# kadircet/ceng795

Measured on AMD Instinct MI355X. Metric: Mrays/s at 1920×1080 (primary+shadow); fraction of HBM roofline, higher is better.
Workload: dtype f32; 1 GPU; C3: 999,698-triangle height field, 1920x1080, 1 point light, primary + shadow rays (BASELINE.json configs[2]); frame=1920x1080, triangles=999698, traversal=fast, parallelism=frames1, frames_in_flight=6

## Files before the change

ceng795_amd/_lib.py:

```python
from __future__ import annotations

import ctypes as C
import os

_HERE = os.path.dirname(os.path.abspath(__file__))
_VARIANT = os.environ.get("CENG795_LIB", "")
LIB_PATH = os.path.join(_HERE, "lib", f"libceng795_rt_{_VARIANT}.so" if _VARIANT else
                        "libceng795_rt.so")

RT_OK = 0
RT_E_INVALID = -1
RT_E_HIP = -2
RT_E_IO = -3
RT_E_PARSE = -4
RT_E_UNSUPPORTED = -5

RT_TRAVERSAL_FAST = 0
RT_TRAVERSAL_REFERENCE = 1

RT_QUERY_REORDER = 1
RT_QUERY_IN_MEDIUM = 2
RT_QUERY_LIGHTS_SHARED = 4
RT_QUERY_NO_SCENE_LIGHTS = 8
RT_QUERY_RAY_TIME = 32
# ... 115 lines not shown
    "rt_set_msaa_seed": (C.c_int, [C.c_void_p, C.c_ulonglong]),
    "rt_render": (C.c_int, [C.c_void_p, C.c_int, C.c_int, C.c_int, C.c_void_p,
                            C.POINTER(rt_stats)]),
    "rt_render_device": (C.c_int, [C.c_void_p, C.c_int, C.c_int, C.c_int, C.c_int, C.c_int,
                                   C.c_int, C.c_void_p, C.c_void_p]),
    "rt_render_device_range": (C.c_int, [C.c_void_p, C.c_int, C.c_int, C.c_int, C.c_int,
                                         C.c_int, C.c_int, C.c_int, C.c_void_p, C.c_void_p]),
    "rt_scene_records_ok": (C.c_int, [C.c_void_p, C.c_int]),
    "rt_tile_costs": (C.c_int, [C.c_void_p, C.c_void_p, C.c_void_p, C.c_int]),
    "rt_resolve_rows": (C.c_int, [C.c_void_p, C.c_int, C.c_int, C.c_int, C.c_void_p, C.c_void_p,
                                  C.c_void_p]),
    "rt_resolve_device": (C.c_int, [C.c_void_p, C.c_int, C.c_int, C.c_int, C.c_int, C.c_int,
                                    C.c_int, C.c_int, C.c_void_p, C.c_void_p, C.c_void_p]),
    "rt_set_kernel_timing": (C.c_int, [C.c_void_p, C.c_int]),
    "rt_read_kernel_times": (C.c_int, [C.c_void_p, C.POINTER(C.c_double),
                                       C.POINTER(C.c_longlong)]),
    "rt_num_tiles": (C.c_int, [C.c_void_p, C.c_int, C.c_int, C.c_int]),
    "rt_collect_stats": (C.c_int, [C.c_void_p, C.POINTER(rt_stats)]),
    "rt_write_png": (C.c_int, [C.c_char_p, C.c_void_p, C.c_int, C.c_int]),
    "rt_camera_from_view": (C.c_int, [C.POINTER(C.c_float), C.POINTER(C.c_float),
                                      C.POINTER(C.c_float), C.POINTER(C.c_float), C.c_float,
                                      C.c_int, C.c_int, C.c_int, C.POINTER(rt_camera)]),
    "rt_last_error": (C.c_char_p, []),
    "rt_abi_version": (C.c_int, []),
    "rt_host_dump_bvh_xml": (C.c_int, [C.c_char_p, C.c_char_p]),
    "rt_host_dump_bvh_desc": (C.c_int, [C.POINTER(rt_scene_desc), C.c_char_p]),
    "rt_host_alloc": (C.c_void_p, [C.c_size_t]),
    "rt_host_free": (None, [C.c_void_p]),
    "rt_host_check_accel_xml": (C.c_int, [C.c_char_p, C.c_int, C.POINTER(C.c_longlong)]),
    "rt_host_accel_slots_check": (C.c_int, [C.c_longlong, C.c_longlong]),
    "rt_host_packet_div": (C.c_int, [C.c_int, C.c_int, C.c_int, C.c_void_p]),
    "rt_host_packet_coords": (C.c_int, [C.c_int] * 8 + [C.c_void_p]),
    "rt_host_accel_slot_hist_xml": (C.c_int, [C.c_char_p, C.c_int, C.POINTER(C.c_longlong)]),
    "rt_debug_counters": (C.c_int, [C.c_void_p, C.POINTER(C.c_longlong)]),
    "rt_debug_timeline": (C.c_longlong, [C.POINTER(C.c_ulonglong), C.c_longlong]),
    "rt_debug_phases": (C.c_longlong, [C.POINTER(C.c_ulonglong), C.c_longlong]),
    "rt_debug_frame_occupancy": (C.c_int, [C.c_int, C.POINTER(C.c_int)]),
    "rt_debug_quotient_check": (C.c_int, [C.c_int, C.c_ulonglong, C.c_longlong,
                                          C.POINTER(C.c_longlong)]),
    "rt_debug_quotient_check_mode": (C.c_int, [C.c_int, C.c_int, C.c_ulonglong, C.c_longlong,
                                               C.POINTER(C.c_longlong)]),
    "rt_ray_query_version": (C.c_int, []),
    "rt_trace_rays_device": (C.c_int, [C.c_void_p, C.c_void_p, C.c_longlong, C.c_void_p, C.c_int,
                                       C.c_void_p]),
    "rt_occluded_device": (C.c_int, [C.c_void_p, C.c_void_p, C.c_longlong, C.c_void_p, C.c_int,
                                     C.c_void_p]),
    "rt_trace_rays": (C.c_int, [C.c_void_p, C.c_void_p, C.c_longlong, C.c_void_p, C.c_int]),
    "rt_occluded": (C.c_int, [C.c_void_p, C.c_void_p, C.c_longlong, C.c_void_p, C.c_int]),
    "rt_host_leaf_objects_desc": (C.c_int, [C.POINTER(rt_scene_desc), C.POINTER(C.c_int), C.c_int]),
    "rt_radiance_query_version": (C.c_int, []),
    "rt_shade_rays_device": (C.c_int, [C.c_void_p, C.c_void_p, C.c_longlong, C.c_int, C.c_void_p,
                                       C.c_int, C.c_void_p]),
    "rt_shade_rays": (C.c_int, [C.c_void_p, C.c_void_p, C.c_longlong, C.c_int, C.c_void_p, C.c_int,
                                C.POINTER(rt_stats)]),
    "rt_set_radiance_scratch_limit": (C.c_int, [C.c_void_p, C.c_size_t]),
    "rt_stream_frame_scratch_bytes": (C.c_longlong, [C.c_void_p, C.c_void_p]),
    "rt_film_version": (C.c_int, []),
    "rt_film_create": (C.c_int, [C.c_void_p, C.c_int, C.c_int, C.c_int, C.c_float,
                                 C.POINTER(C.c_void_p)]),
    "rt_film_destroy": (None, [C.c_void_p]),
    "rt_film_clear_device": (C.c_int, [C.c_void_p, C.c_void_p]),
    "rt_film_splat_device": (C.c_int, [C.c_void_p, C.c_void_p, C.c_void_p, C.c_longlong,
                                       C.c_void_p]),
    "rt_film_shade_rays_device": (C.c_int, [C.c_void_p, C.c_void_p, C.c_void_p, C.c_longlong,
                                            C.c_int, C.c_int, C.c_void_p]),
    "rt_film_resolve_device": (C.c_int, [C.c_void_p, C.c_void_p, C.c_void_p]),
# ... 106 lines not shown
```

ceng795_amd/csrc/accel_build.cpp:

```cpp
#include <algorithm>
#include <array>
#include <cmath>
#include <cstdio>
#include <cstdlib>
#include <cstring>
#include <limits>
#include <stdexcept>
#include <vector>

#include "host_scene.h"

namespace rt {
namespace {

struct Box {
  float lo[3] = {std::numeric_limits<float>::infinity(), std::numeric_limits<float>::infinity(),
                 std::numeric_limits<float>::infinity()};
  float hi[3] = {-std::numeric_limits<float>::infinity(), -std::numeric_limits<float>::infinity(),
                 -std::numeric_limits<float>::infinity()};
  void grow(const float* b) {
    for (int a = 0; a < 3; a++) {
      lo[a] = std::min(lo[a], b[a]);
      hi[a] = std::max(hi[a], b[a + 3]);
    }
// ... 147 lines not shown
  return f;
}

void two_sum(double a, double b, double& s, double& e) {
  s = a + b;
  const double bb = s - a;
  e = (a - (s - bb)) + (b - bb);
}

double add_down(double a, double b) {
  double s, e;
  two_sum(a, b, s, e);
  return e < 0.0 ? std::nextafter(s, -INFINITY) : s;
}

double add_up(double a, double b) {
  double s, e;
  two_sum(a, b, s, e);
  return e > 0.0 ? std::nextafter(s, INFINITY) : s;
}

bool sum_le(double a, double b, double c, double d) {
  double s1, e1, s2, e2;
  two_sum(a, b, s1, e1);
  two_sum(c, d, s2, e2);
  return s1 != s2 ? s1 < s2 : e1 <= e2;
}

struct Slot {
  int ref;
  Box box;
};

void encode_node(DevNode8& W, const Slot* sl, int n, const double* margin) {
  double lo[3] = {INFINITY, INFINITY, INFINITY}, hi[3] = {-INFINITY, -INFINITY, -INFINITY};
  for (int k = 0; k < n; k++)
    for (int a = 0; a < 3; a++) {
      lo[a] = std::min(lo[a], add_down((double)sl[k].box.lo[a], -margin[a]));
      hi[a] = std::max(hi[a], add_up((double)sl[k].box.hi[a], margin[a]));
    }
  W.scale = 0;
  int ka[3];
  for (int a = 0; a < 3; a++) {
    W.origin[a] = float_down(lo[a]);
    const double ext = add_up(hi[a], -(double)W.origin[a]);
    int k = (int)std::ceil(std::log2(std::max(ext, 1e-300) / 32768.0));
    k = std::min(std::max(k, -120), 120);
    while (std::ldexp(ext, -k) > 32768.0) k++;
    if (k > 127) throw std::runtime_error("culling node extent beyond the fp16 scale range");
    ka[a] = k;
    W.scale |= (uint32_t)(uint8_t)(int8_t)k << (8 * a);
  }
  for (int c = 0; c < kWideSlots; c++)
    for (int a = 0; a < 3; a++) {
      if (c >= n) {
        W.box[c][a] = (uint32_t)kHalfNaN | ((uint32_t)kHalfNaN << 16);
        continue;
      }
      const double o = (double)W.origin[a];
      const double pl = add_down(add_down((double)sl[c].box.lo[a], -margin[a]), -o);
      const double ph = add_up(add_up((double)sl[c].box.hi[a], margin[a]), -o);
      const uint16_t l = half_dir(std::ldexp(pl, -ka[a]), false);
      const uint16_t h = half_dir(std::ldexp(ph, -ka[a]), true);
      W.box[c][a] = (uint32_t)l | ((uint32_t)h << 16);
    }
}

void decode_slot(const DevNode8& W, int c, double* lo, double* hi) {
  for (int a = 0; a < 3; a++) {
    const int k = (int)(int8_t)(uint8_t)((W.scale >> (8 * a)) & 255);
    lo[a] = std::ldexp(half_value((uint16_t)(W.box[c][a] & 0xffff)), k);
    hi[a] = std::ldexp(half_value((uint16_t)(W.box[c][a] >> 16)), k);
  }
}

bool holds_with_margin(double origin, double lo, double hi, double glo, double ghi, double margin) {
  return sum_le(origin, lo, glo, -margin) && sum_le(ghi, margin, origin, hi);
}

#ifndef RT_WIDE_NODE_COST
#define RT_WIDE_NODE_COST 1.0
#endif
#ifndef RT_WIDE_LEAF_COST
#define RT_WIDE_LEAF_COST 0.3
#endif
#ifndef RT_WIDE_SLOT_COST
#define RT_WIDE_SLOT_COST 0.0
#endif
constexpr double kNodeCost = RT_WIDE_NODE_COST, kLeafCost = RT_WIDE_LEAF_COST,
                 kSlotCost = RT_WIDE_SLOT_COST;

struct WideCollapse {
  const SahBuilder& B;
  std::vector<std::array<double, kWideSlots + 1>> F;
// ... 42 lines not shown
  void emit_side(int n, int s, int k, std::vector<Slot>& out) const {
    const int c = B.nodes[n].child[s];
    if (k == 1 || c < 0) {
      out.push_back(Slot{c, B.nodes[n].box[s]});
      return;
    }
    emit(c, k, out);
  }
  void emit(int n, int k, std::vector<Slot>& out) const {
    const int k1 = split[n][k];
    emit_side(n, 0, k1, out);
    emit_side(n, 1, k - k1, out);
  }
};

int collapse_wide(HostScene& s, const SahBuilder& B, int broot, const std::vector<int>& holder,
                  const std::vector<float>& ref_box) {
  const std::vector<Item>& items = B.items;
  const WideCollapse W8(B, broot);
  struct Job {
    int bnode, wide;
  };
  const int w0 = (int)s.nodes.size();
  s.nodes.resize(w0 + 2);
  std::vector<Job> todo{{broot, w0}};
  std::vector<int> order;
  std::vector<std::vector<int>> kids;
  std::vector<Slot> slots;
  while (!todo.empty()) {
    const Job j = todo.back();
    todo.pop_back();
    slots.clear();
    W8.emit(j.bnode, W8.tk[j.bnode], slots);
    const int n = (int)slots.size();
    const Slot* sl = slots.data();
    DevNode8 W;
    std::memset(&W, 0, sizeof W);
    encode_node(W, sl, n, s.cull_margin);
    int inner = 0;
    for (int k = 0; k < n; k++) inner += sl[k].ref >= 0;
    W.inner_base = inner ? (int)s.nodes.size() : 0;
    s.nodes.resize(s.nodes.size() + 2 * (size_t)inner);
    W.leaf_base = (int)s.leaves.size();
    std::vector<int> mine;
    int off = 0, r = 0;
    for (int k = 0; k < n; k++) {
      W.kinds |= kSlotValid << k;
      if (sl[k].ref >= 0) {
        mine.push_back(W.inner_base + 2 * r++);
        continue;
      }
      const Item& it = items[~sl[k].ref];
      W.kinds |= kSlotLeafy << k;
      if (it.pair) W.kinds |= kSlotPair << k;
      W.offs |= (uint32_t)off << (4 * k);
      for (int q = 0; q < (it.pair ? 2 : 1); q++) {
        const int l = it.leaf + q;
        const DevPrim& p = s.prims[l];
        DevLeaf L;
        std::memcpy(L.v0, p.v0, sizeof L.v0);
        std::memcpy(L.a1, p.a1, sizeof L.a1);
        std::memcpy(L.a2, p.a2, sizeof L.a2);
        L.dfs = l | (p.kind == kPrimSphere ? kLeafSphere : 0);
        const float* g = &ref_box[(size_t)holder[l] * 6];
        L.g0 = g[0], L.g1 = g[1], L.g2 = g[2], L.g3 = g[3], L.g4 = g[4], L.g5 = g[5];
        s.leaves.push_back(L);
        off++;
      }
    }
    std::memcpy(&s.nodes[j.wide], &W, sizeof W);
    order.push_back(j.wide);
    kids.push_back(mine);
    r = 0;
    std::vector<Job> next;
    for (int k = 0; k < n; k++)
      if (sl[k].ref >= 0) next.push_back({sl[k].ref, mine[r++]});
    for (auto it = next.rbegin(); it != next.rend(); ++it) todo.push_back(*it);
  }
  std::vector<int> need(s.nodes.size(), 0);
  for (size_t i = order.size(); i-- > 0;) {
    int deepest = 0;
    for (int c : kids[i]) deepest = std::max(deepest, need[c]);
    need[order[i]] = kids[i].empty() ? 0 : (int)kids[i].size() - 1 + deepest;
  }
  s.accel_depth = need[w0] + 1;
  return w0 | kWideTag;
}

void add_octant_copies(HostScene& s, size_t nref, size_t nw) {
  s.accel_stride = (int)nw;
  s.nodes.resize(nref + (size_t)kOctantCopies * nw);
  for (int k = 1; k < kOctantCopies; k++)
    for (size_t i = 0; i < nw; i += 2) {
      DevNode8 W;
      std::memcpy(&W, &s.nodes[nref + i], sizeof W);
      if ((unsigned)W.kinds & ~((unsigned)W.kinds >> 8) & 0xffu) W.inner_base += k * (int)nw;
      for (int c = 0; c < kWideSlots; c++)
        for (int x = 0; x < 3; x++)
          if (k >> x & 1) W.box[c][x] = W.box[c][x] << 16 | W.box[c][x] >> 16;
      std::memcpy(&s.nodes[nref + (size_t)k * nw + i], &W, sizeof W);
    }
}

}

std::string accel_slots_error(size_t ref_slots, size_t wide_slots) {
  const size_t total = ref_slots + (size_t)kOctantCopies * wide_slots;
  if (total < kMaxNodeSlots) return "";
  return "scene too large for the culling tree: " + std::to_string(ref_slots) +
// ... 63 lines not shown
  };
  std::vector<int> todo{0};
  while (!todo.empty()) {
    const int n = todo.back();
    todo.pop_back();
    const DevNode& N = s.nodes[n];
    if (K == 2 && N.child[0] < 0 && N.child[1] < 0) {
      if (~N.child[1] != ~N.child[0] + 1) throw std::logic_error("leaf children not consecutive");
      push_item(~N.child[0], true, n);
      continue;
    }
    for (int side = 0; side < 2; side++) {
      const int c = N.child[side];
      if (c < 0)
        push_item(~c, false, n);
      else
        todo.push_back(c);
    }
  }
  SahBuilder B{items, {}};
  const int broot = B.build(0, (int)items.size());
  Box u;
  for (const Item& it : items) u.grow(it.box);
  for (int a = 0; a < 3; a++) {
    s.accel_box[a] = u.lo[a] - std::fabs(u.lo[a]) * 0x1p-20f - 0x1p-100f;
    s.accel_box[a + 3] = u.hi[a] + std::fabs(u.hi[a]) * 0x1p-20f + 0x1p-100f;
  }
  s.accel_items = (int)items.size();
  s.accel_root = collapse_wide(s, B, broot, holder, ref_box);
  const size_t nref = (size_t)(s.accel_root & ~kWideTag), nw = s.nodes.size() - nref;
  const std::string err = accel_slots_error(nref, nw);
  if (!err.empty()) throw std::domain_error(err);
  add_octant_copies(s, nref, nw);
}

std::string check_accel(const HostScene& s, int K, long long stats[4]) {
  for (int i = 0; i < 4; i++) stats[i] = 0;
  if (s.accel_root < 0) return "";
  K = std::min(K, 2);
  const int nref = s.accel_root & ~kWideTag;
  const size_t nleaf = s.prims.size();
  for (int n = 0; n < nref; n++) {
    const DevNode& N = s.nodes[n];
    if (N.pad != 0) return "reference node " + std::to_string(n) + " is flagged";
    for (int side = 0; side < 2; side++) {
      const int c = N.child[side];
      if (c >= 0) {
        if (c >= nref || s.ancestry[c].parent != n) return "bad parent of node " + std::to_string(c);
        for (int a = 0; a < 3; a++)
          if (s.ancestry[c].box[a] != N.lo[a][side] || s.ancestry[c].box[a + 3] != N.hi[a][side])
            return "ancestry box of node " + std::to_string(c) + " differs from its slot";
      } else if ((size_t)~c >= nleaf || s.ancestry[~c].leaf_parent != n) {
        return "bad holder of leaf " + std::to_string(~c);
      }
    }
  }
  for (int a = 0; a < 6; a++)
    if (s.ancestry[0].box[a] != s.root_box[a]) return "root box differs from ancestry";
  if (s.leaves.size() != nleaf) return "culling leaves do not cover the leaves once";
  std::vector<int> seen(nleaf, 0);
  long long lone = 0, items = 0, nodes = 0;
  const double* mg = s.cull_margin;
  struct Frame {
    int node, depth;
  };
  if (s.accel_stride <= 0) return "octant copies and their stride disagree";
  const size_t ncull = (size_t)s.accel_stride;
  if (s.nodes.size() != (size_t)nref + (size_t)kOctantCopies * ncull || ncull % 2)
    return "node array is not the reference nodes and " + std::to_string(kOctantCopies) +
           " copies of the culling nodes";
  if (!accel_slots_error((size_t)nref, ncull).empty()) return "node array past the offset limit";
  std::vector<Frame> todo{{s.accel_root, 1}};
  std::vector<int> order;
  std::vector<double> ulo(s.nodes.size() * 3, INFINITY), uhi(s.nodes.size() * 3, -INFINITY);
  while (!todo.empty()) {
    const Frame f = todo.back();
    todo.pop_back();
    if (!(f.node & kWideTag)) return "culling child is not a wide node";
    const int idx = f.node & ~kWideTag;
    if (idx < nref || (size_t)idx + 1 >= (size_t)nref + ncull) return "wide node index out of range";
    DevNode8 W;
    std::memcpy(&W, &s.nodes[idx], sizeof W);
    nodes++;
    order.push_back(idx);
    stats[2] = std::max<long long>(stats[2], f.depth);
    int valid = 0, r = 0;
    const unsigned vbits = (unsigned)W.kinds & 0xffu;
    if (vbits & (vbits + 1)) return "valid slots not first";
    for (int c = 0; c < kWideSlots; c++) {
      if (!(W.kinds & (kSlotValid << c))) {
        if (W.box[c][0] != (0x7e00u | 0x7e000000u)) return "invalid slot without NaN planes";
        continue;
      }
      valid++;
      double lo[3], hi[3];
      decode_slot(W, c, lo, hi);
      if (!(W.kinds & (kSlotLeafy << c))) {
        if (W.kinds & (kSlotPair << c)) return "pair flag on an inner slot";
        const int child = W.inner_base + 2 * r++;
        todo.push_back({child | kWideTag, f.depth + 1});
        continue;
      }
      items++;
      const bool pair = (W.kinds & (kSlotPair << c)) != 0;
      const int first = W.leaf_base + (int)((W.offs >> (4 * c)) & 15);
      if (first < 0 || (size_t)first + (pair ? 2 : 1) > s.leaves.size()) return "leaf range out of bounds";
      if (!pair) lone++;
      if (pair && K < 2) return "leaf pair with K = 1";
      int hold = -1;
      for (int q = 0; q < (pair ? 2 : 1); q++) {
        const DevLeaf& L = s.leaves[first + q];
        const int l = L.dfs & ~kLeafSphere;
        if (l < 0 || (size_t)l >= nleaf) return "leaf index out of range";
        if (seen[l]++) return "leaf " + std::to_string(l) + " in two treelets";
        const DevPrim& p = s.prims[l];
        if ((p.kind == kPrimSphere) != ((L.dfs & kLeafSphere) != 0) ||
            std::memcmp(L.v0, p.v0, 12) || std::memcmp(L.a1, p.a1, 12) || std::memcmp(L.a2, p.a2, 12))
          return "leaf record differs from its primitive";
        const int h = s.ancestry[l].leaf_parent;
        const float g[6] = {L.g0, L.g1, L.g2, L.g3, L.g4, L.g5};
        if (std::memcmp(g, s.ancestry[h].box, sizeof g)) return "guard box is not the holder's box";
        if (q == 0) hold = h;
        if (q == 1 && (h != hold || l != (s.leaves[first].dfs & ~kLeafSphere) + 1 ||
                       s.nodes[h].child[0] != ~(l - 1) || s.nodes[h].child[1] != ~l))
          return "leaf pair " + std::to_string(l - 1) + " is not one node's two leaves";
        if (q == 0 && pair && s.nodes[h].child[0] != ~l) return "leaf pair does not start its holder";
        for (int a = 0; a < 3; a++)
          if (!holds_with_margin(W.origin[a], lo[a], hi[a], g[a], g[a + 3], mg[a]))
            return "slot box does not hold its guard box with the margin";
      }
    }
    if (valid < 2) return "wide node with fewer than two slots";
  }
  for (size_t l = 0; l < nleaf; l++)
    if (!seen[l]) return "leaf " + std::to_string(l) + " in no treelet";
  for (auto it = order.rbegin(); it != order.rend(); ++it) {
    DevNode8 W;
    std::memcpy(&W, &s.nodes[*it], sizeof W);
    double nlo[3] = {INFINITY, INFINITY, INFINITY}, nhi[3] = {-INFINITY, -INFINITY, -INFINITY};
    int r = 0;
    for (int c = 0; c < kWideSlots; c++) {
      if (!(W.kinds & (kSlotValid << c))) continue;
      double lo[3], hi[3];
      decode_slot(W, c, lo, hi);
      double glo[3], ghi[3];
      if (W.kinds & (kSlotLeafy << c)) {
        const DevLeaf& L = s.leaves[W.leaf_base + ((W.offs >> (4 * c)) & 15)];
        const float g[6] = {L.g0, L.g1, L.g2, L.g3, L.g4, L.g5};
        for (int a = 0; a < 3; a++) glo[a] = g[a], ghi[a] = g[a + 3];
      } else {
        const size_t ci = (size_t)(W.inner_base + 2 * r++) * 3;
        for (int a = 0; a < 3; a++) {
          glo[a] = ulo[ci + a];
          ghi[a] = uhi[ci + a];
          if (!holds_with_margin(W.origin[a], lo[a], hi[a], glo[a], ghi[a], mg[a]))
            return "culling box does not hold the guard boxes below it with the margin";
        }
      }
      for (int a = 0; a < 3; a++) {
        nlo[a] = std::min(nlo[a], glo[a]);
        nhi[a] = std::max(nhi[a], ghi[a]);
      }
    }
    for (int a = 0; a < 3; a++) {
      ulo[(size_t)*it * 3 + a] = nlo[a];
      uhi[(size_t)*it * 3 + a] = nhi[a];
    }
  }
  const size_t r0 = (size_t)nref * 3;
  for (int a = 0; a < 3; a++)
    if (s.accel_box[a] > ulo[r0 + a] || s.accel_box[a + 3] < uhi[r0 + a])
      return "culling root box does not contain the tree";
  for (int k = 1; k < kOctantCopies; k++)
    for (size_t i = 0; i < ncull; i += 2) {
      DevNode8 W, C;
      std::memcpy(&W, &s.nodes[nref + i], sizeof W);
      std::memcpy(&C, &s.nodes[nref + (size_t)k * ncull + i], sizeof C);
      const bool has_inner = ((unsigned)W.kinds & ~((unsigned)W.kinds >> 8) & 0xffu) != 0;
      if (C.inner_base != W.inner_base + (has_inner ? k * (int)ncull : 0))
        return "octant copy " + std::to_string(k) + ": inner_base not shifted by k * stride";
      for (int c = 0; c < kWideSlots; c++)
        for (int x = 0; x < 3; x++) {
          const uint32_t w = W.box[c][x];
          if (C.box[c][x] != ((k >> x & 1) ? (w << 16 | w >> 16) : w))
            return "octant copy " + std::to_string(k) + ": slot word halves not as its octant's";
        }
      C.inner_base = W.inner_base;
      std::memcpy(C.box, W.box, sizeof C.box);
      if (std::memcmp(&C, &W, sizeof W))
        return "octant copy " + std::to_string(k) + " differs from copy 0 outside the planes";
    }
  stats[0] = items;
  stats[1] = nodes;
  stats[3] = lone;
  return "";
}

void accel_slot_histogram(const HostScene& s, long long hist[kWideSlots + 1]) {
  for (int i = 0; i <= kWideSlots; i++) hist[i] = 0;
  if (s.accel_root < 0) return;
  std::vector<int> todo{s.accel_root & ~kWideTag};
  while (!todo.empty()) {
    const int idx = todo.back();
    todo.pop_back();
    DevNode8 W;
    std::memcpy(&W, &s.nodes[idx], sizeof W);
    int valid = 0, r = 0;
    for (int c = 0; c < kWideSlots; c++) {
      if (!(W.kinds & (kSlotValid << c))) continue;
      valid++;
      if (!(W.kinds & (kSlotLeafy << c))) todo.push_back(W.inner_base + 2 * r++);
    }
    hist[valid]++;
  }
}

}
```

ceng795_amd/csrc/host_scene.h:

```cpp
#ifndef CENG795_HOST_SCENE_H_
#define CENG795_HOST_SCENE_H_

#include <string>
#include <vector>

#include "../../include/ceng795_rt.h"
#include "rt_internal.h"

namespace rt {

struct LeafSource {
  int kind;
  int i0, i1, i2;
  float center[3], radius;
  int material;
  int object;
};

struct HostScene {
  float background[3] = {0, 0, 0};
  float ambient[3] = {0, 0, 0};
  float eps = 0.001f;
  int max_depth = 0;
  std::vector<DevMaterial> materials;
// ... 1 lines not shown
  std::vector<rt_camera> cameras;
  std::vector<std::string> image_names;
  std::vector<DevNode> nodes;
  std::vector<DevPrim> prims;
  std::vector<float> normals;
  std::vector<LeafSource> leaf_src;
  std::vector<int> leaf_object;
  int root_kind = kRootNode;
  int root_ref = 0;
  float root_box[6] = {0, 0, 0, 0, 0, 0};
  int depth = 0;
  int accel_root = -1;
  int accel_depth = 0;
  int accel_items = 0;
  int accel_stride = 0;
  float accel_box[6] = {0, 0, 0, 0, 0, 0};
  double cull_margin[3] = {0, 0, 0};
  std::vector<DevLeaf> leaves;
  std::vector<DevAncestry> ancestry;
  int quot_ok = 0;
  bool smooth = false;
  std::vector<int> leaf_tri;
  std::vector<float> vertex_normals;
  std::vector<float> vertex_uv;
};

void host_vertex_normals(const rt_scene_desc& desc, float* out);
void build_surface(const rt_scene_desc& desc, const rt_surface_desc* surf, HostScene& s);

void build_accel(HostScene& s, int K);
std::string accel_slots_error(size_t ref_slots, size_t wide_slots);
std::string check_accel(const HostScene& s, int K, long long stats[4]);
void accel_slot_histogram(const HostScene& s, long long hist[kWideSlots + 1]);

void build_host_scene(const rt_scene_desc& desc, HostScene& out);

void build_host_globals(const rt_scene_desc& desc, HostScene& out);

struct InstHost {
  std::vector<HostScene> meshes;
  std::vector<int> mesh_leaf_base;
  std::vector<int> mesh_object_base;
  std::vector<long long> accel_stats;
  std::vector<DevInstance> instances;
  std::vector<float> inverse;
  std::vector<int> inst_top_dfs;
  std::vector<DevNode> top_nodes;
  std::vector<DevPrim> top_prims;
  std::vector<float> top_normals;
  std::vector<int> top_info;
  int top_root_kind = kTopNode;
  int top_depth = 0;
  int top_quot_ok = 1;
  float top_box[6] = {0, 0, 0, 0, 0, 0};
  bool has_spheres = false;
  int leaves = 0;
  bool has_motion = false;
  std::vector<DevMotionInstance> motion_instances;
  std::vector<DevMotionSphere> motion_spheres;
  std::vector<float> sphere_inverse;
  std::vector<float> sphere_box;
  std::vector<int> object_top_dfs;
};
void build_instanced(const rt_scene_desc& desc, const rt_instance_desc& inst, int treelets,
                     InstHost& out);
void build_moving(const rt_scene_desc& desc, const rt_instance_desc* inst,
// ... 38 lines not shown
```

ceng795_amd/csrc/rt_api.hip:

```cpp
#include <hip/hip_runtime.h>
#include <rccl/rccl.h>

#include <algorithm>
#include <cmath>
#include <array>
#include <atomic>
#include <cstdio>
#include <cstdlib>
#include <cstring>
#include <exception>
#include <memory>
#include <mutex>
#include <new>
#include <optional>
#include <stdexcept>
#include <string>
#include <vector>

#include "../../include/ceng795_rt.h"
#include "hip_host.h"
#include "host_scene.h"
#include "rt_internal.h"

namespace rt {
// ... 1930 lines not shown
int rt_host_check_accel_xml(const char* xml_path, int treelet_leaves, long long* stats4) {
  if (!xml_path || !stats4) return set_error(RT_E_INVALID, "rt_host_check_accel_xml: NULL argument");
  return guarded([&] {
    XmlSceneStorage st;
    rt_scene_desc d;
    load_scene_xml(xml_path, st, d);
    HostScene h;
    build_host_scene(d, h);
    build_accel(h, treelet_leaves);
    const std::string err = check_accel(h, treelet_leaves, stats4);
    if (!err.empty()) throw std::invalid_argument("culling tree: " + err);
    return RT_OK;
  });
}

int rt_host_accel_slot_hist_xml(const char* xml_path, int treelet_leaves, long long* hist9) {
  if (!xml_path || !hist9)
    return set_error(RT_E_INVALID, "rt_host_accel_slot_hist_xml: NULL argument");
  return guarded([&] {
    XmlSceneStorage st;
    rt_scene_desc d;
    load_scene_xml(xml_path, st, d);
    HostScene h;
    build_host_scene(d, h);
    build_accel(h, treelet_leaves);
    long long stats[4];
    const std::string err = check_accel(h, treelet_leaves, stats);
    if (!err.empty()) throw std::invalid_argument("culling tree: " + err);
    accel_slot_histogram(h, hist9);
    return RT_OK;
  });
}

int rt_host_accel_slots_check(long long ref_slots, long long wide_slots) {
  if (ref_slots < 0 || wide_slots < 0)
    return set_error(RT_E_INVALID, "rt_host_accel_slots_check: bad argument");
  const std::string err = accel_slots_error((size_t)ref_slots, (size_t)wide_slots);
  return err.empty() ? RT_OK : set_error(RT_E_UNSUPPORTED, err);
}

int rt_host_packet_div(int divisor, int first, int count, int* quot) {
  if (divisor < 1 || first < 0 || count < 0 || (long long)first + count > (1ll << 31) || !quot)
    return set_error(RT_E_INVALID, "rt_host_packet_div: bad argument");
  const DivMagic m = div_magic(divisor);
  for (int i = 0; i < count; i++) quot[i] = div_by((int)((long long)first + i), m);
  return RT_OK;
}

int rt_host_packet_coords(int tiles_x, int num_sel_tiles, int tile_begin, int tile_step,
                          int block_deal, int order_regions, int order_stride, int count,
                          int* out4) {
  if (tiles_x < 1 || num_sel_tiles < 0 || tile_begin < 0 || tile_step < 1 || order_regions < 1 ||
      order_stride < 0 || count < 0 || !out4)
    return set_error(RT_E_INVALID, "rt_host_packet_coords: bad argument");
  RenderParams P;
  std::memset(&P, 0, sizeof P);
  P.tiles_x = tiles_x;
  P.num_sel_tiles = num_sel_tiles;
  P.tile_begin = tile_begin;
  P.tile_step = tile_step;
  P.block_deal = block_deal ? 1 : 0;
  P.order_regions = order_regions;
  P.order_stride = order_stride;
  P.tile_block = whole_tile_rows(P);
  const PacketGeom G = packet_geom(P);
  for (int p = 0; p < count; p++) {
// ... 776 lines not shown
```

ceng795_amd/csrc/rt_internal.h:

```cpp
#ifndef CENG795_RT_INTERNAL_H_
#define CENG795_RT_INTERNAL_H_

#include <stdint.h>

namespace rt {

constexpr int kTile = 8;
constexpr int kWavesPerBlock = 4;
constexpr int kLaneStack = 64;
constexpr int kCounterRows = 64;
constexpr int kCounterWidth = 16;
enum : int {
  kCntPrimary = 0, kCntShadow = 1, kCntSecondary = 2, kCntHits = 3,
  kCntPrimNodes = 4, kCntPrimNodeLanes = 5, kCntPrimLeaves = 6, kCntPrimLeafLanes = 7,
  kCntShadNodes = 8, kCntShadNodeLanes = 9, kCntShadLeaves = 10, kCntShadLeafLanes = 11,
  kCntExactBox = 12,
  kCntGuardTests = 13,
  kCntPrimWide = 14, kCntShadWide = 15
};

enum : int {
  kPhVisits = 0, kPhSlotsTested = 1, kPhSlotHits = 2, kPhLeafyHits = 3, kPhPairHits = 4,
  kPhInnerHits = 5, kPhPushes = 6, kPhPops = 7, kPhFlushes = 8, kPhFlushIters = 9,
  kPhaseEvents = 10
};
enum : int {
  kPhCycPrimTotal = 2 * kPhaseEvents, kPhCycPrimVisit, kPhCycPrimLoad, kPhCycPrimFlush,
  kPhCycShadTotal, kPhCycShadVisit, kPhCycShadLoad, kPhCycShadFlush, kPhCycShade,
  kPhCycFrame, kPhWaves,
  kPhCarryZero, kPhCarryLow, kPhCarryHigh,
  kPhDeferPrim, kPhDeferShad = kPhDeferPrim + 4,
  kPhOctPrimPackets = kPhDeferShad + 4, kPhOctPrimWalks, kPhOctShadPackets, kPhOctShadWalks,
  kPhCycPrologue, kPhCycPrimSetup, kPhCycPrimWalk, kPhCycPrimTail, kPhCycShadSetup,
  kPhCycShadWalk, kPhCycShadTail,
  kPhCycShadeRecord, kPhCycShadeLoads, kPhCycShadeMath,
  kPhaseSlots
};
enum : int {
  kDfSurvivors = 0, kDfGuardIters = 1, kDfSplitDrains = 2, kDfRejected = 3, kDeferEvents = 4
};

constexpr int kDefaultTreeletLeaves = 2;

struct alignas(16) DevNode {
  float lo[3][2];
  float hi[3][2];
  int32_t child[2];
  int32_t axis;
  int32_t pad;
};
static_assert(sizeof(DevNode) == 64, "node must be one 64-byte scalar load");

constexpr int32_t kWideTag = 1 << 30;
constexpr int kOctantCopies = 8;
constexpr size_t kMaxNodeSlots = size_t(1) << 26;
constexpr int kWideSlots = 8;
enum : int32_t { kSlotValid = 1, kSlotLeafy = 1 << 8, kSlotPair = 1 << 16 };
struct alignas(16) DevNode8 {
  float origin[3];
  uint32_t scale;
  int32_t inner_base;
  int32_t leaf_base;
  int32_t kinds;
  uint32_t offs;
  uint32_t box[kWideSlots][3];
};
static_assert(sizeof(DevNode8) == 128, "a wide node is two s_load_dwordx16");
static_assert(sizeof(DevNode8) == 2 * 64, "a wide node is two node slots");

constexpr int32_t kLeafSphere = 1 << 30;
struct alignas(16) DevLeaf {
  float v0[3];
  int32_t dfs;
  float a1[3];
  float g0;
  float a2[3];
  float g1;
  float g2, g3, g4, g5;
};
static_assert(sizeof(DevLeaf) == 64, "leaf record is four 16-byte loads");

enum PrimKind : int32_t { kPrimTriangle = 0, kPrimSphere = 1 };

struct alignas(16) DevPrim {
  float v0[3];
  float a1[3];
  float a2[3];
  int32_t kind;
  int32_t material;
  float cx;
// ... 461 lines not shown
```

ceng795_amd/csrc/rt_kernels.hip:

```cpp
#include <hip/hip_runtime.h>

#include <cstddef>
#include <cstdint>
#include <type_traits>
#include <vector>

#include "rt_internal.h"

#pragma clang fp contract(off)

namespace rt {

#define RT_INF __builtin_huge_valf()
constexpr float kEps = 0.000001f;

constexpr int kCounterSlots = kCounterRows;

#ifdef RT_DIAG
#define DIAG(stmt) stmt
#else
#define DIAG(stmt)
#endif
struct Diag {
  unsigned long long nodes = 0, node_lanes = 0, leaves = 0, leaf_lanes = 0, wide = 0, guard = 0;
// ... 738 lines not shown
                                           Diag& dg) {
  v16i a, b;
  DIAG(const unsigned long long tl0 = clock_now());
  load_node8(nodes, node, a, b);
  DIAG(dg.cyc_load += clock_now() - tl0);
  const unsigned scale = (unsigned)a[3];
  const int inner_base = a[4], leaf_base = a[5], kinds = a[6];
  const unsigned offs = (unsigned)a[7];
  const unsigned inner = (unsigned)kinds & ~((unsigned)kinds >> 8) & 0xffu;
  DIAG(dg.nodes++; dg.wide++; dg.node_lanes += __builtin_popcountll(m));
  const float o[3] = {r.o.x, r.o.y, r.o.z}, rc[3] = {r.r.x, r.r.y, r.r.z}, mg[3] = {r.m.x, r.m.y, r.m.z};
  [[maybe_unused]] const int sh[3] = {r.sh0, r.sh1, r.sh2};
  float S[3], Alo[3], Ahi[3];
#pragma unroll
  for (int x = 0; x < 3; x++) {
    S[x] = __builtin_amdgcn_ldexpf(rc[x], (int)(signed char)(scale >> (8 * x)));
    const float A = __int_as_float(a[x]) - o[x];
    Alo[x] = __builtin_fmaf(A, rc[x], -__builtin_fabsf(mg[x]));
    Ahi[x] = __builtin_fmaf(A, rc[x], __builtin_fabsf(mg[x]));
    if (SKIP) {
      const bool sk = x == 0 ? r.skip0 : (x == 1 ? r.skip1 : r.skip2);
      S[x] = sk ? 0.0f : S[x];
      Alo[x] = sk ? -RT_INF : Alo[x];
      Ahi[x] = sk ? RT_INF : Ahi[x];
    }
  }
  {
    const bool in = lane_in(m);
    S[0] = in ? S[0] : 1.0f;
    Ahi[0] = in ? Ahi[0] : -RT_INF;
  }
  int nxt = -1;
  uint64_t nm = 0;
  unsigned inner_bits = inner;
  asm("" : "+s"(inner_bits));
#pragma unroll
  for (int c = 0; c < kWideSlots; c++) {
    if (!(kinds & (kSlotValid << c))) break;
    DIAG(dg.ev[kPhSlotsTested]++);
    float n3[3], f3[3];
#pragma unroll
    for (int x = 0; x < 3; x++) {
      int w = RT_NODE_WORD(8 + 3 * c + x);
      if (!COHERENT)
        w = (int)__builtin_amdgcn_alignbit((unsigned)w, (unsigned)w, (unsigned)sh[x]);
      n3[x] = __builtin_fmaf(half_lo(w), S[x], Alo[x]);
      f3[x] = __builtin_fmaf(half_hi(w), S[x], Ahi[x]);
    }
    const float tn = __builtin_fmaxf(__builtin_fmaxf(n3[0], n3[1]), n3[2]);
    const float tf = __builtin_fminf(__builtin_fminf(f3[0], f3[1]), f3[2]);
    const uint64_t hm = lanes_ge(tf, __builtin_fmaxf(tn, 0.0f));
    if (hm) {
      DIAG(dg.ev[kPhSlotHits]++);
      if (kinds & (kSlotLeafy << c)) {
        DIAG(dg.ev[kPhLeafyHits]++);
        const int leaf = leaf_base + (int)((offs >> (4 * c)) & 15u);
        [[maybe_unused]] const bool pair = (kinds & (kSlotPair << c)) != 0;
        DIAG(dg.ev[kPhPairHits] += pair);
        batch_push_n<!SHADOW>(L, pending, leaf, hm, ((unsigned)kinds >> (16 + c)) & 1u);
        DIAG(dg.leaves += 1 + pair; dg.leaf_lanes += (1 + pair) * __builtin_popcountll(hm));
      }
      if (inner_bits & (1u << c)) {
        const int ch = (inner_base + 2 * __builtin_popcount(inner & ((1u << c) - 1u))) | kWideTag;
        DIAG(dg.ev[kPhInnerHits]++);
        if (nxt < 0) {
          nxt = ch;
          nm = hm;
        } else {
          st.push(ch, hm);
        }
      }
    }
  }
  if (nxt >= 0) {
    node = nxt;
    m = nm;
    return true;
  }
  return st.pop_live(node, m, alive);
}
#undef RT_NODE_WORD

#ifndef RT_PRIO_V
#define RT_PRIO_V 3
#endif
#ifndef RT_PRIO_F
#define RT_PRIO_F 0
#endif
#ifndef RT_PRIO_REST
#define RT_PRIO_REST 1
#endif
#define RT_PRIO_VISIT_BEGIN __builtin_amdgcn_s_setprio(RT_PRIO_V)
#define RT_PRIO_VISIT_END __builtin_amdgcn_s_setprio(RT_PRIO_REST)
#define RT_PRIO_FLUSH_BEGIN __builtin_amdgcn_s_setprio(RT_PRIO_F)
#define RT_PRIO_FLUSH_END __builtin_amdgcn_s_setprio(RT_PRIO_REST)
template <bool SKIP, bool FAST, bool DEEP, bool SPHERES, bool CAMERA = false, bool OCT = false>
__device__ __forceinline__ void closest_hit(const RenderParams& P, const DevNode* __restrict__ nodes,
                                            int* spill, WaveLeafLds& L, const LaneRay& r,
                                            bool active, float& best_t, int& best_leaf, Diag& dg,
                                            int root_off = 0) {
  static_assert(!OCT || FAST, "octant copies exist of the culling nodes only");
  if (!OCT) {
    best_t = RT_INF;
    best_leaf = -1;
// ... 2745 lines not shown
```

include/ceng795_rt.h:

```cpp
#ifndef CENG795_RT_H_
#define CENG795_RT_H_
#include <stddef.h>
#ifdef __cplusplus
extern "C" {
#endif

#define CENG795_RT_ABI_VERSION 7

enum {
  RT_OK = 0,
  RT_E_INVALID = -1,
  RT_E_HIP = -2,
  RT_E_IO = -3,
  RT_E_PARSE = -4,
  RT_E_UNSUPPORTED = -5
};

typedef struct rt_material {
  float ambient[3];
  float diffuse[3];
  float specular[3];
  float mirror[3];
  float transparency[3];
  float refraction_index;
// ... 55 lines not shown
  long long primary_rays;
  long long shadow_rays;
  long long secondary_rays;
  long long primary_hits;
  double kernel_ms;
} rt_stats;

enum {
  RT_TRAVERSAL_FAST = 0,
  RT_TRAVERSAL_REFERENCE = 1
};
typedef struct rt_scene rt_scene;

int rt_scene_create(const rt_scene_desc* desc, int device, rt_scene** out);
void rt_scene_destroy(rt_scene* scene);

int rt_scene_load_xml(const char* xml_path, int device, rt_scene** out);

int rt_scene_create_multi(const rt_scene_desc* desc, int device_count, const int* devices,
                          rt_scene** out);
int rt_scene_load_xml_multi(const char* xml_path, int device_count, const int* devices,
                            rt_scene** out);
int rt_scene_device_count(const rt_scene* scene);

int rt_scene_num_cameras(const rt_scene* scene);
int rt_scene_camera(const rt_scene* scene, int camera_index, rt_camera* out);
const char* rt_scene_image_name(const rt_scene* scene, int camera_index);
int rt_scene_num_lights(const rt_scene* scene);
int rt_scene_dump_bvh(const rt_scene* scene, const char* path);
int rt_host_dump_bvh_xml(const char* xml_path, const char* out_path);
int rt_host_dump_bvh_desc(const rt_scene_desc* desc, const char* out_path);
int rt_host_check_accel_xml(const char* xml_path, int treelet_leaves, long long* stats4);
int rt_host_accel_slot_hist_xml(const char* xml_path, int treelet_leaves, long long* hist9);
int rt_host_accel_slots_check(long long ref_slots, long long wide_slots);
int rt_host_packet_div(int divisor, int first, int count, int* quot);
int rt_host_packet_coords(int tiles_x, int num_sel_tiles, int tile_begin, int tile_step,
                          int block_deal, int order_regions, int order_stride, int count,
                          int* out4);
int rt_scene_bvh_depth(const rt_scene* scene);

int rt_set_traversal(rt_scene* scene, int mode);

int rt_render(rt_scene* scene, int camera_index, int starting_row, int row_stride,
              float* out_rgb, rt_stats* stats);

void* rt_host_alloc(size_t bytes);
void rt_host_free(void* ptr);

enum { RT_TILE_MAJOR = 1, RT_TILE_BLOCKS = 2,
       RT_TILE_RECORDS = 4   };

int rt_render_device(rt_scene* scene, int camera_index, int starting_row, int row_stride,
                     int tile_begin, int tile_step, int tile_major, float* d_out,
                     void* hip_stream);
int rt_render_device_range(rt_scene* scene, int camera_index, int starting_row, int row_stride,
                           int tile_begin, int tile_step, int tile_count, int tile_major,
                           float* d_out, void* hip_stream);
int rt_untile_device(rt_scene* scene, int camera_index, int starting_row, int row_stride,
                     int devices, int slot, int tile_offset, int flags, const float* d_gathered,
                     float* d_out, void* hip_stream);
enum { RT_UNTILE_BLOCKS = 1,
       RT_UNTILE_SKIP_ROOT = 2   };
int rt_scene_records_ok(const rt_scene* scene, int camera_index);
int rt_resolve_device(rt_scene* scene, int camera_index, int starting_row, int row_stride,
                      int devices, int slot, int tile_offset, int flags,
                      const unsigned* d_gathered, float* d_out, void* hip_stream);
// ... 198 lines not shown
```

Baseline: 16040 Mrays/s.

## Pack inner slots from slot 0 and leaf slots down from slot 7 in wide nodes

The wide BVH node builder now places inner children contiguously from slot 0 and leaf children contiguously down from slot 7, and records both counts in the kinds word. Traversal then runs two separate unrolled loops, one for inner slots and one for leaf slots. The child index becomes inner_base + 2*c instead of a popcount, and the per-slot leafy/inner branching goes away. This aims to cut divergent branching and scalar overhead in the slot loop. The price is a different child visitation order and two loops that may raise code size. Validation helpers and a kind histogram API are added.

```diff
diff --git a/ceng795_amd/_lib.py b/ceng795_amd/_lib.py
--- a/ceng795_amd/_lib.py
+++ b/ceng795_amd/_lib.py
@@ -171,6 +171,8 @@
     "rt_host_packet_div": (C.c_int, [C.c_int, C.c_int, C.c_int, C.c_void_p]),
     "rt_host_packet_coords": (C.c_int, [C.c_int] * 8 + [C.c_void_p]),
     "rt_host_accel_slot_hist_xml": (C.c_int, [C.c_char_p, C.c_int, C.POINTER(C.c_longlong)]),
+    "rt_host_accel_kind_hist_xml": (C.c_int, [C.c_char_p, C.c_int, C.POINTER(C.c_longlong)]),
+    "rt_host_check_wide_node": (C.c_int, [C.c_void_p, C.c_ulonglong]),
     "rt_debug_counters": (C.c_int, [C.c_void_p, C.POINTER(C.c_longlong)]),
     "rt_debug_timeline": (C.c_longlong, [C.POINTER(C.c_ulonglong), C.c_longlong]),
     "rt_debug_phases": (C.c_longlong, [C.POINTER(C.c_ulonglong), C.c_longlong]),
diff --git a/ceng795_amd/csrc/accel_build.cpp b/ceng795_amd/csrc/accel_build.cpp
--- a/ceng795_amd/csrc/accel_build.cpp
+++ b/ceng795_amd/csrc/accel_build.cpp
@@ -203,12 +203,12 @@
   Box box;
 };
 
-void encode_node(DevNode8& W, const Slot* sl, int n, const double* margin) {
+void encode_node(DevNode8& W, const Slot* const at[kWideSlots], const double* margin) {
   double lo[3] = {INFINITY, INFINITY, INFINITY}, hi[3] = {-INFINITY, -INFINITY, -INFINITY};
-  for (int k = 0; k < n; k++)
-    for (int a = 0; a < 3; a++) {
-      lo[a] = std::min(lo[a], add_down((double)sl[k].box.lo[a], -margin[a]));
-      hi[a] = std::max(hi[a], add_up((double)sl[k].box.hi[a], margin[a]));
+  for (int c = 0; c < kWideSlots; c++)
+    for (int a = 0; at[c] && a < 3; a++) {
+      lo[a] = std::min(lo[a], add_down((double)at[c]->box.lo[a], -margin[a]));
+      hi[a] = std::max(hi[a], add_up((double)at[c]->box.hi[a], margin[a]));
     }
   W.scale = 0;
   int ka[3];
@@ -224,13 +224,13 @@
   }
   for (int c = 0; c < kWideSlots; c++)
     for (int a = 0; a < 3; a++) {
-      if (c >= n) {
+      if (!at[c]) {
         W.box[c][a] = (uint32_t)kHalfNaN | ((uint32_t)kHalfNaN << 16);
         continue;
       }
       const double o = (double)W.origin[a];
-      const double pl = add_down(add_down((double)sl[c].box.lo[a], -margin[a]), -o);
-      const double ph = add_up(add_up((double)sl[c].box.hi[a], margin[a]), -o);
+      const double pl = add_down(add_down((double)at[c]->box.lo[a], -margin[a]), -o);
+      const double ph = add_up(add_up((double)at[c]->box.hi[a], margin[a]), -o);
       const uint16_t l = half_dir(std::ldexp(pl, -ka[a]), false);
       const uint16_t h = half_dir(std::ldexp(ph, -ka[a]), true);
       W.box[c][a] = (uint32_t)l | ((uint32_t)h << 16);
@@ -339,28 +339,32 @@
     todo.pop_back();
     slots.clear();
     W8.emit(j.bnode, W8.tk[j.bnode], slots);
-    const int n = (int)slots.size();
-    const Slot* sl = slots.data();
+    const Slot* at[kWideSlots] = {};
+    int inner = 0, leafy = 0;
+    for (const Slot& sl : slots)
+      if (sl.ref >= 0)
+        at[inner++] = &sl;
+      else
+        at[kWideSlots - 1 - leafy++] = &sl;
     DevNode8 W;
     std::memset(&W, 0, sizeof W);
-    encode_node(W, sl, n, s.cull_margin);
-    int inner = 0;
-    for (int k = 0; k < n; k++) inner += sl[k].ref >= 0;
+    encode_node(W, at, s.cull_margin);
     W.inner_base = inner ? (int)s.nodes.size() : 0;
     s.nodes.resize(s.nodes.size() + 2 * (size_t)inner);
     W.leaf_base = (int)s.leaves.size();
+    W.kinds = (int32_t)((uint32_t)inner << kSlotInnerCountShift |
+                        (uint32_t)leafy << kSlotLeafyCountShift);
     std::vector<int> mine;
-    int off = 0, r = 0;
-    for (int k = 0; k < n; k++) {
-      W.kinds |= kSlotValid << k;
-      if (sl[k].ref >= 0) {
-        mine.push_back(W.inner_base + 2 * r++);
-        continue;
-      }
-      const Item& it = items[~sl[k].ref];
-      W.kinds |= kSlotLeafy << k;
-      if (it.pair) W.kinds |= kSlotPair << k;
-      W.offs |= (uint32_t)off << (4 * k);
+    for (int c = 0; c < inner; c++) {
+      W.kinds |= kSlotValid << c;
+      mine.push_back(W.inner_base + 2 * c);
+    }
+    int off = 0;
+    for (int c = kWideSlots - 1; c >= kWideSlots - leafy; c--) {
+      const Item& it = items[~at[c]->ref];
+      W.kinds |= (kSlotValid | kSlotLeafy) << c;
+      if (it.pair) W.kinds |= kSlotPair << c;
+      W.offs |= (uint32_t)off << (4 * c);
       for (int q = 0; q < (it.pair ? 2 : 1); q++) {
         const int l = it.leaf + q;
         const DevPrim& p = s.prims[l];
@@ -378,10 +382,8 @@
     std::memcpy(&s.nodes[j.wide], &W, sizeof W);
     order.push_back(j.wide);
     kids.push_back(mine);
-    r = 0;
     std::vector<Job> next;
-    for (int k = 0; k < n; k++)
-      if (sl[k].ref >= 0) next.push_back({sl[k].ref, mine[r++]});
+    for (int c = 0; c < inner; c++) next.push_back({at[c]->ref, mine[c]});
     for (auto it = next.rbegin(); it != next.rend(); ++it) todo.push_back(*it);
   }
   std::vector<int> need(s.nodes.size(), 0);
@@ -511,6 +513,26 @@
   const std::string err = accel_slots_error(nref, nw);
   if (!err.empty()) throw std::domain_error(err);
   add_octant_copies(s, nref, nw);
+}
+
+std::string wide_slot_order_error(const DevNode8& W) {
+  const unsigned valid = (unsigned)W.kinds & 0xffu, leafy = (unsigned)W.kinds >> 8 & 0xffu;
+  const unsigned pair = (unsigned)W.kinds >> 16 & 0xffu, inner = valid & ~leafy;
+  if (leafy & ~valid) return "leafy flag on an invalid slot";
+  if (pair & ~leafy) return "pair flag on a slot that is not leafy";
+  const int ni = __builtin_popcount(inner), nl = __builtin_popcount(leafy);
+  if ((unsigned)W.kinds >> kSlotInnerCountShift != ((unsigned)ni | (unsigned)nl << 4))
+    return "slot counts differ from the slot bits";
+  if (inner & (inner + 1u)) {
+    const unsigned below_top = (1u << (31 - __builtin_clz(inner))) - 1u;
+    return leafy & below_top ? "leafy slot below an inner one"
+                             : "inner slots not contiguous from slot 0";
+  }
+  if (leafy != (0xffu & ~(0xffu >> nl))) return "leafy slots not contiguous down from slot 7";
+  for (int c = 0; c < kWideSlots; c++)
+    if (!(valid >> c & 1) && W.box[c][0] != (0x7e00u | 0x7e000000u))
+      return "invalid slot without NaN planes";
+  return "";
 }
 
 std::string check_accel(const HostScene& s, int K, long long stats[4]) {
@@ -563,20 +585,16 @@
     nodes++;
     order.push_back(idx);
     stats[2] = std::max<long long>(stats[2], f.depth);
-    int valid = 0, r = 0;
-    const unsigned vbits = (unsigned)W.kinds & 0xffu;
-    if (vbits & (vbits + 1)) return "valid slots not first";
+    int valid = 0;
+    const std::string order_err = wide_slot_order_error(W);
+    if (!order_err.empty()) return order_err;
     for (int c = 0; c < kWideSlots; c++) {
-      if (!(W.kinds & (kSlotValid << c))) {
-        if (W.box[c][0] != (0x7e00u | 0x7e000000u)) return "invalid slot without NaN planes";
-        continue;
-      }
+      if (!(W.kinds & (kSlotValid << c))) continue;
       valid++;
       double lo[3], hi[3];
       decode_slot(W, c, lo, hi);
       if (!(W.kinds & (kSlotLeafy << c))) {
-        if (W.kinds & (kSlotPair << c)) return "pair flag on an inner slot";
-        const int child = W.inner_base + 2 * r++;
+        const int child = W.inner_base + 2 * c;
         todo.push_back({child | kWideTag, f.depth + 1});
         continue;
       }
@@ -617,7 +635,6 @@
     DevNode8 W;
     std::memcpy(&W, &s.nodes[*it], sizeof W);
     double nlo[3] = {INFINITY, INFINITY, INFINITY}, nhi[3] = {-INFINITY, -INFINITY, -INFINITY};
-    int r = 0;
     for (int c = 0; c < kWideSlots; c++) {
       if (!(W.kinds & (kSlotValid << c))) continue;
       double lo[3], hi[3];
@@ -628,7 +645,7 @@
         const float g[6] = {L.g0, L.g1, L.g2, L.g3, L.g4, L.g5};
         for (int a = 0; a < 3; a++) glo[a] = g[a], ghi[a] = g[a + 3];
       } else {
-        const size_t ci = (size_t)(W.inner_base + 2 * r++) * 3;
+        const size_t ci = (size_t)(W.inner_base + 2 * c) * 3;
         for (int a = 0; a < 3; a++) {
           glo[a] = ulo[ci + a];
           ghi[a] = uhi[ci + a];
@@ -684,14 +701,30 @@
     todo.pop_back();
     DevNode8 W;
     std::memcpy(&W, &s.nodes[idx], sizeof W);
-    int valid = 0, r = 0;
+    int valid = 0;
     for (int c = 0; c < kWideSlots; c++) {
       if (!(W.kinds & (kSlotValid << c))) continue;
       valid++;
-      if (!(W.kinds & (kSlotLeafy << c))) todo.push_back(W.inner_base + 2 * r++);
+      if (!(W.kinds & (kSlotLeafy << c))) todo.push_back(W.inner_base + 2 * c);
     }
     hist[valid]++;
   }
 }
 
-}
+void accel_kind_histogram(const HostScene& s, long long hist[(kWideSlots + 1) * (kWideSlots + 1)]) {
+  for (int i = 0; i < (kWideSlots + 1) * (kWideSlots + 1); i++) hist[i] = 0;
+  if (s.accel_root < 0) return;
+  std::vector<int> todo{s.accel_root & ~kWideTag};
+  while (!todo.empty()) {
+    const int idx = todo.back();
+    todo.pop_back();
+    DevNode8 W;
+    std::memcpy(&W, &s.nodes[idx], sizeof W);
+    const unsigned leafy = (unsigned)W.kinds >> 8 & 0xffu, inner = (unsigned)W.kinds & ~leafy & 0xffu;
+    for (int c = 0; c < kWideSlots; c++)
+      if (inner >> c & 1) todo.push_back(W.inner_base + 2 * c);
+    hist[__builtin_popcount(inner) * (kWideSlots + 1) + __builtin_popcount(leafy)]++;
+  }
+}
+
+}
diff --git a/ceng795_amd/csrc/host_scene.h b/ceng795_amd/csrc/host_scene.h
--- a/ceng795_amd/csrc/host_scene.h
+++ b/ceng795_amd/csrc/host_scene.h
@@ -57,6 +57,8 @@
 std::string accel_slots_error(size_t ref_slots, size_t wide_slots);
 std::string check_accel(const HostScene& s, int K, long long stats[4]);
 void accel_slot_histogram(const HostScene& s, long long hist[kWideSlots + 1]);
+void accel_kind_histogram(const HostScene& s, long long hist[(kWideSlots + 1) * (kWideSlots + 1)]);
+std::string wide_slot_order_error(const DevNode8& W);
 
 void build_host_scene(const rt_scene_desc& desc, HostScene& out);
 
diff --git a/ceng795_amd/csrc/rt_api.hip b/ceng795_amd/csrc/rt_api.hip
--- a/ceng795_amd/csrc/rt_api.hip
+++ b/ceng795_amd/csrc/rt_api.hip
@@ -1986,6 +1986,36 @@
   });
 }
 
+int rt_host_accel_kind_hist_xml(const char* xml_path, int treelet_leaves, long long* hist81) {
+  if (!xml_path || !hist81)
+    return set_error(RT_E_INVALID, "rt_host_accel_kind_hist_xml: NULL argument");
+  return guarded([&] {
+    XmlSceneStorage st;
+    rt_scene_desc d;
+    load_scene_xml(xml_path, st, d);
+    HostScene h;
+    build_host_scene(d, h);
+    build_accel(h, treelet_leaves);
+    long long stats[4];
+    const std::string err = check_accel(h, treelet_leaves, stats);
+    if (!err.empty()) throw std::invalid_argument("culling tree: " + err);
+    accel_kind_histogram(h, hist81);
+    return RT_OK;
+  });
+}
+
+int rt_host_check_wide_node(const void* node, unsigned long long bytes) {
+  if (!node || bytes != sizeof(DevNode8))
+    return set_error(RT_E_INVALID, "rt_host_check_wide_node: NULL node or not 128 bytes");
+  return guarded([&] {
+    DevNode8 W;
+    std::memcpy(&W, node, sizeof W);
+    const std::string err = wide_slot_order_error(W);
+    if (!err.empty()) throw std::invalid_argument("wide node: " + err);
+    return RT_OK;
+  });
+}
+
 int rt_host_accel_slots_check(long long ref_slots, long long wide_slots) {
   if (ref_slots < 0 || wide_slots < 0)
     return set_error(RT_E_INVALID, "rt_host_accel_slots_check: bad argument");
diff --git a/ceng795_amd/csrc/rt_internal.h b/ceng795_amd/csrc/rt_internal.h
--- a/ceng795_amd/csrc/rt_internal.h
+++ b/ceng795_amd/csrc/rt_internal.h
@@ -56,6 +56,7 @@
 constexpr size_t kMaxNodeSlots = size_t(1) << 26;
 constexpr int kWideSlots = 8;
 enum : int32_t { kSlotValid = 1, kSlotLeafy = 1 << 8, kSlotPair = 1 << 16 };
+constexpr int kSlotInnerCountShift = 24, kSlotLeafyCountShift = 28;
 struct alignas(16) DevNode8 {
   float origin[3];
   uint32_t scale;
diff --git a/ceng795_amd/csrc/rt_kernels.hip b/ceng795_amd/csrc/rt_kernels.hip
--- a/ceng795_amd/csrc/rt_kernels.hip
+++ b/ceng795_amd/csrc/rt_kernels.hip
@@ -794,16 +794,11 @@
   }
   int nxt = -1;
   uint64_t nm = 0;
-  unsigned inner_bits = inner;
-  asm("" : "+s"(inner_bits));
-#pragma unroll
-  for (int c = 0; c < kWideSlots; c++) {
-    if (!(kinds & (kSlotValid << c))) break;
-    DIAG(dg.ev[kPhSlotsTested]++);
+  auto slot_lanes = [&](const int (&w3)[3]) -> uint64_t {
     float n3[3], f3[3];
 #pragma unroll
     for (int x = 0; x < 3; x++) {
-      int w = RT_NODE_WORD(8 + 3 * c + x);
+      int w = w3[x];
       if (!COHERENT)
         w = (int)__builtin_amdgcn_alignbit((unsigned)w, (unsigned)w, (unsigned)sh[x]);
       n3[x] = __builtin_fmaf(half_lo(w), S[x], Alo[x]);
@@ -811,27 +806,39 @@
     }
     const float tn = __builtin_fmaxf(__builtin_fmaxf(n3[0], n3[1]), n3[2]);
     const float tf = __builtin_fminf(__builtin_fminf(f3[0], f3[1]), f3[2]);
-    const uint64_t hm = lanes_ge(tf, __builtin_fmaxf(tn, 0.0f));
+    return lanes_ge(tf, __builtin_fmaxf(tn, 0.0f));
+  };
+  const int child0 = inner_base | kWideTag;
+#pragma unroll
+  for (int c = 0; c < kWideSlots; c++) {
+    if (!(inner & (1u << c))) break;
+    DIAG(dg.ev[kPhSlotsTested]++);
+    const int w3[3] = {RT_NODE_WORD(8 + 3 * c), RT_NODE_WORD(9 + 3 * c), RT_NODE_WORD(10 + 3 * c)};
+    const uint64_t hm = slot_lanes(w3);
     if (hm) {
-      DIAG(dg.ev[kPhSlotHits]++);
-      if (kinds & (kSlotLeafy << c)) {
-        DIAG(dg.ev[kPhLeafyHits]++);
-        const int leaf = leaf_base + (int)((offs >> (4 * c)) & 15u);
-        [[maybe_unused]] const bool pair = (kinds & (kSlotPair << c)) != 0;
-        DIAG(dg.ev[kPhPairHits] += pair);
-        batch_push_n<!SHADOW>(L, pending, leaf, hm, ((unsigned)kinds >> (16 + c)) & 1u);
-        DIAG(dg.leaves += 1 + pair; dg.leaf_lanes += (1 + pair) * __builtin_popcountll(hm));
+      DIAG(dg.ev[kPhSlotHits]++; dg.ev[kPhInnerHits]++);
+      const int ch = child0 + 2 * c;
+      if (nxt < 0) {
+        nxt = ch;
+        nm = hm;
+      } else {
+        st.push(ch, hm);
       }
-      if (inner_bits & (1u << c)) {
-        const int ch = (inner_base + 2 * __builtin_popcount(inner & ((1u << c) - 1u))) | kWideTag;
-        DIAG(dg.ev[kPhInnerHits]++);
-        if (nxt < 0) {
-          nxt = ch;
-          nm = hm;
-        } else {
-          st.push(ch, hm);
-        }
-      }
+    }
+  }
+#pragma unroll
+  for (int c = kWideSlots - 1; c >= 0; c--) {
+    if (!(kinds & (kSlotLeafy << c))) break;
+    DIAG(dg.ev[kPhSlotsTested]++);
+    const int w3[3] = {RT_NODE_WORD(8 + 3 * c), RT_NODE_WORD(9 + 3 * c), RT_NODE_WORD(10 + 3 * c)};
+    const uint64_t hm = slot_lanes(w3);
+    if (hm) {
+      DIAG(dg.ev[kPhSlotHits]++; dg.ev[kPhLeafyHits]++);
+      const int leaf = leaf_base + (int)((offs >> (4 * c)) & 15u);
+      [[maybe_unused]] const bool pair = (kinds & (kSlotPair << c)) != 0;
+      DIAG(dg.ev[kPhPairHits] += pair);
+      batch_push_n<!SHADOW>(L, pending, leaf, hm, ((unsigned)kinds >> (16 + c)) & 1u);
+      DIAG(dg.leaves += 1 + pair; dg.leaf_lanes += (1 + pair) * __builtin_popcountll(hm));
     }
   }
   if (nxt >= 0) {
diff --git a/include/ceng795_rt.h b/include/ceng795_rt.h
--- a/include/ceng795_rt.h
+++ b/include/ceng795_rt.h
@@ -111,6 +111,8 @@
 int rt_host_dump_bvh_desc(const rt_scene_desc* desc, const char* out_path);
 int rt_host_check_accel_xml(const char* xml_path, int treelet_leaves, long long* stats4);
 int rt_host_accel_slot_hist_xml(const char* xml_path, int treelet_leaves, long long* hist9);
+int rt_host_accel_kind_hist_xml(const char* xml_path, int treelet_leaves, long long* hist81);
+int rt_host_check_wide_node(const void* node, unsigned long long bytes);
 int rt_host_accel_slots_check(long long ref_slots, long long wide_slots);
 int rt_host_packet_div(int divisor, int first, int count, int* quot);
 int rt_host_packet_coords(int tiles_x, int num_sel_tiles, int tile_begin, int tile_step,
```

Result: faster. 16560 Mrays/s, median of 6 (+3.2%).
